# DDMAL/text_alignment

Hardware: AMD Instinct MI355X
Metric: nw_dp_cells_per_s (higher is better)
Workload: dtype int32; 1 GPU; affine-gap NW, 4096 problems of 4096x4096 per GPU per step, default scoring [8,-4,-7,-7,-3,0], two-phase (score fill + windowed traceback); parallelism=problems sharded x1, no data-path collective, distinct_problems=256

## Files before the change

### text_alignment_amd/csrc/nw_band.h

```cpp
#pragma once
#include <stdint.h>

#include "nw_cell.h"

namespace ta {

constexpr int kBandSentinel = -(1 << 24);
constexpr int kBandMaxLen = 32768;
static_assert(((int64_t)kBandSentinel - 2ll * kBandMaxLen * 128 - (1 << 21)) * 64 > INT32_MIN, "sentinel-derived values, encoded");
struct BandRange { int gl, gh; };
TA_HD BandRange band_groups(int n, int m, int w, int s) {
    const int ngroups = PtrLayout<4>::ngroups(m);
    const int lo = (m < n ? m - n : 0) - w, hi = (m > n ? m - n : 0) + w;
    const int i0 = s * 256 + 1;
    const int jmin = i0 + lo > 1 ? i0 + lo : 1;
    const int jmax = i0 + 255 + hi < m ? i0 + 255 + hi : m;
    const int kmin = jmin - 1, kmax = jmax - 1 + 63;
    int gl = kmin >= 2 ? ((kmin - 2) / 64) * 16 - 16 : 0;
    if (gl < 0) gl = 0;
    int gh = (kmax / 64) * 16 + 32;
    if (gh >= ngroups || gh <= gl) gh = ngroups;
    if (gl >= gh) gl = 0;
    return BandRange{gl, gh};
}
// ... 51 lines not shown
    const int off_lo = m < n ? m - n : 0, off_hi = m > n ? m - n : 0;
    const int lo = wl < w_outer ? off_lo - (int)wl : off_lo - w_outer;
    const int hi = wh < w_outer ? off_hi + (int)wh : off_hi + w_outer;
    const int i0 = s * 256 + 1;
    const int jmin = i0 + lo > 1 ? i0 + lo : 1;
    const int jmax = i0 + 255 + hi < m ? i0 + 255 + hi : m;
    const int kmin = jmin - 1, kmax = jmax - 1 + 63;
    int gl = kmin >= 2 ? ((kmin - 2) / 64) * 16 - 16 : 0;
    if (gl < 0) gl = 0;
    int gh = (kmax / 64) * 16 + 32;
    if (gh >= ngroups || gh <= gl) gh = ngroups;
    if (gl >= gh) gl = 0;
    return BandRange{gl, gh};
}
template <int PM = kFunnelFullPm>
TA_HD bool funnel_ok(int n, int m, const FunnelSys& f, int w_outer) {
    const int nstrips = PtrLayout<4>::nstrips(n), ngroups = PtrLayout<4>::ngroups(m);
    BandRange prev{0, 0};
    for (int s = 0; s < nstrips; ++s) {
        const BandRange r = funnel_raw<PM>(n, m, f, w_outer, s);
        if (r.gl < 0) return false;
        if (s > 0) {
            if (r.gl < prev.gl || r.gh < prev.gh) return false;
            if (r.gl > 0 && prev.gh < ngroups && 4 * r.gl + 2 > 4 * prev.gh - 63) return false;
        }
        prev = r;
    }
    return true;
}
TA_HD BandRange funnel_groups(int n, int m, const int32_t* prm, int w_outer, int s) {
    const FunnelSys f = funnel_sys(prm);
    return funnel_ok(n, m, f, w_outer) ? funnel_raw(n, m, f, w_outer, s) : band_groups(n, m, w_outer, s);
}
template <int PM = kFunnelFullPm>
inline bool funnel_ranges(int n, int m, const int32_t* prm, int w_outer, BandRange* rg) {
    const FunnelSys f = funnel_sys(prm);
    const bool own = funnel_ok<PM>(n, m, f, w_outer);
    const int nstrips = PtrLayout<4>::nstrips(n);
    for (int s = 0; s < nstrips; ++s) rg[s] = own ? funnel_raw<PM>(n, m, f, w_outer, s) : band_groups(n, m, w_outer, s);
    return own;
}

TA_HD int funnel_jlo(const BandRange& r, int i) { return r.gl == 0 ? 1 : 4 * r.gl - ((i - 1) % 256) / 4 + 3; }
TA_HD int funnel_jhi(const BandRange& r, int i, int m) {
    if (r.gh == PtrLayout<4>::ngroups(m)) return m;
    const int j = 4 * r.gh - ((i - 1) % 256) / 4;
    return j < m ? j : m;
}
inline int64_t funnel_exit0(int n, int m, const int32_t* prm, const BandRange* rg) {
    const FunnelSys f = funnel_sys(prm);
    int64_t best = -(1ll << 40);
    auto out = [&](int i, int j) {
        if (i < 1 || i > n || j < 1 || j > m) return false;
        const BandRange& r = rg[(i - 1) / 256];
        return j < funnel_jlo(r, i) || j > funnel_jhi(r, i, m);
    };
    auto take = [&](int64_t db, int i, int j) {
        if (out(i, j)) best = bmax(best, db + f.ap + funnel_suf<int64_t>(n - i, m - j, f));
    };
    for (int j = 0; j <= m; ++j) { take(-j, 1, j); take(-j, 1, j + 1); }
    for (int i = 1; i <= n; ++i) { take(-i, i, 1); take(-i, i + 1, 1); }
    return best;
}

struct FunnelLcs { int mat, mis; };
TA_HD FunnelLcs funnel_lcs_sys(const int32_t* prm) { return FunnelLcs{prm[0], prm[1]}; }
template <typename T>
TA_HD T funnel_suf_lcs(T rn, T rm, T l, const FunnelSys& f, const FunnelLcs& q) {
    const T stat = funnel_suf<T>(rn, rm, f);
    if (q.mis >= q.mat) return stat;
    const T d = rn < rm ? rn : rm;
    const T lp = l < d ? (l < 0 ? 0 : l) : d;
    const T none = rn * (T)f.cvi + rm * (T)f.chi;
    const T all_match = lp * (T)q.mat + (rn - lp) * (T)f.cvi + (rm - lp) * (T)f.chi;
    const T most = lp * (T)q.mat + (d - lp) * (T)q.mis + (rn - d) * (T)f.cvi + (rm - d) * (T)f.chi;
    T best = none > all_match ? none : all_match;
    if (most > best) best = most;
    return best < stat ? best : stat;
}

constexpr int kLcsMaxM = 4096;
constexpr int kLcsMaxAlphabet = 64;

TA_HD int lcs_row_off(int max_n) { return (max_n + 1 + 63) & ~63; }
TA_HD int64_t lcs_stride(int max_n) { return (int64_t)lcs_row_off(max_n) + 192ll * PtrLayout<4>::nstrips(max_n); }
TA_HD int lcs_row_at(const int32_t* row, int m, int j) {
    const int c = m - j;
    if (c <= 0) return 0;
    const int w = c >> 6, b = c & 63;
    if (w >= 64) return row[128 + 63] + __builtin_popcountll(((const uint64_t*)row)[63]);
    const uint64_t bits = ((const uint64_t*)row)[w];
    return row[128 + w] + (b ? __builtin_popcountll(bits & ((1ull << b) - 1)) : 0);
}

struct LcsRun { int t0, w, s, l, b, count; };
struct LcsRunCursor { int s, l; };
TA_HD LcsRunCursor lcs_run_begin(int n) { return LcsRunCursor{PtrLayout<4>::nstrips(n), -1}; }
template <typename GhOf>
TA_HD LcsRun lcs_next_run(int n, int m, int ngroups, LcsRunCursor& c, GhOf&& gh_of) {
    while (true) {
        if (c.l < 0) {
            if (--c.s < 0) return LcsRun{INT32_MAX, 0, 0, 0, 0, 0};
            const int top = (n - 256 * c.s - 1) >> 2;
            c.l = top < 63 ? top : 63;
        }
        const int gh = gh_of(c.s);
        const int lmin = 4 * gh > m ? 4 * gh - m : 0;
        if (gh >= ngroups || c.l < lmin) { c.l = -1; continue; }
        const int cnt = m - 4 * gh + c.l, b = cnt & 63, left = c.l - lmin + 1;
        const LcsRun r{n - 256 * c.s - 4 * c.l - 1 + (cnt >> 6), cnt >> 6, c.s, c.l, b, b + 1 < left ? b + 1 : left};
        c.l = r.count == left ? -1 : c.l - r.count;
        return r;
    }
}

}
```

### text_alignment_amd/csrc/ta_nw2.hip

```cpp
#include <hip/hip_runtime.h>
#include <stdint.h>
#include <array>
#include <atomic>
#include <map>
#include <type_traits>
#include <vector>

#include "nw_band.h"
#include "nw_cell.h"
#include "nw_hw.h"
#include "ta_common.h"

namespace ta {

#ifndef TA_CK_GROUPS
#define TA_CK_GROUPS 16
#endif
constexpr int kCkGroups = TA_CK_GROUPS;
static_assert(kCkGroups % 4 == 0 && kCkGroups >= 4, "whole blocks of four groups");
constexpr int kStateInts = 10;
constexpr int kWsRange = 0x7ffff000;

#ifndef TA_SUBROWS
#define TA_SUBROWS 2
// ... 483 lines not shown
                            rowp[col] = make_int2(kBandSentinel, kBandSentinel);
                    }
                }
                if (W > 1) {
                    asm volatile("s_waitcnt vmcnt(0)" ::: "memory");
                    if (lane == 63)
                        __hip_atomic_store(&prog[wave], pass * ngroups + ngroups, __ATOMIC_RELEASE,
                                           __HIP_MEMORY_SCOPE_WORKGROUP);
                }
            }
        }
        for (; g < g_fin; ++g) group_edge(g);
        patch(false);
    }
    if constexpr (FUNNEL) {
        if (lane == 0 && cnt_wave > 0) {
            atomicMax(&a.band_cert[kCertWords * p + 1], ex_wave);
            atomicAdd(&a.band_cert[kCertWords * p + 2], cnt_wave);
        }
    }
}

__global__ __launch_bounds__(256) void nw_band_cert_init_kernel(NwArgs a, const int32_t* x0) {
    const int p = blockIdx.x * 256 + threadIdx.x;
    if (p >= a.nprob) return;
    const int n = (int)(a.t_off[p + 1] - a.t_off[p]), m = (int)(a.o_off[p + 1] - a.o_off[p]);
    const bool own = n > 0 && m > 0 && n <= kBandMaxLen && m <= kBandMaxLen &&
                     funnel_ok(n, m, funnel_sys(a.params + (size_t)p * a.params_stride), a.band_w);
    a.band_cert[kCertWords * p] = INT32_MIN;
    a.band_cert[kCertWords * p + 1] = x0[p];
    a.band_cert[kCertWords * p + 2] = 0;
    a.band_cert[kCertWords * p + 3] = own ? 1 : 0;
    a.band_ok[p] = 0;
}
__global__ __launch_bounds__(256) void nw_band_certify_kernel(NwArgs a) {
    const int p = blockIdx.x * 256 + threadIdx.x;
    if (p >= a.nprob) return;
    const int n = (int)(a.t_off[p + 1] - a.t_off[p]);
    const int32_t* c = a.band_cert + kCertWords * (size_t)p;
    const bool ok = n > 0 && c[2] == PtrLayout<4>::nstrips(n) && c[0] > a.band_u[p] && c[0] > c[1];
    a.band_ok[p] = ok ? 1 : 0;
}

__global__ __launch_bounds__(256) void nw_band_cert_init_lcs_kernel(NwArgs a, const int32_t* x0, int alphabet) {
    const int p = blockIdx.x * 256 + threadIdx.x;
    if (p >= a.nprob) return;
    const int n = (int)(a.t_off[p + 1] - a.t_off[p]), m = (int)(a.o_off[p + 1] - a.o_off[p]);
    const int32_t* prm = a.params + (size_t)p * a.params_stride;
    const FunnelSys f = funnel_sys(prm);
    const bool sized = n > 0 && m > 0 && n <= kBandMaxLen && m <= kBandMaxLen;
    const bool lcs = sized && n >= 2 && m <= kLcsMaxM && n <= a.lcs_max_n && alphabet > 0 && alphabet <= kLcsMaxAlphabet &&
                     prm[0] > prm[1] && funnel_ok<kFunnelLcsScalePm>(n, m, f, a.band_w);
    const bool own = lcs || (sized && funnel_ok(n, m, f, a.band_w));
    a.band_cert[kCertWords * p] = INT32_MIN;
    a.band_cert[kCertWords * p + 1] = lcs ? -(1 << 30) : x0[p];
    a.band_cert[kCertWords * p + 2] = lcs ? -1 : 0;
    a.band_cert[kCertWords * p + 3] = lcs ? 2 : own ? 1 : 0;
    a.band_ok[p] = 0;
}

#ifndef TA_LCS_PROFILE
#define TA_LCS_PROFILE 0
#endif
#if TA_LCS_PROFILE
#define LCS_PROFILE_DECL long long pc_t = __builtin_readcyclecounter(), pc_setup = 0, pc_steps = 0, pc_events = 0, pc_tail = 0;
#define LCS_LAP(acc) { const long long now_ = __builtin_readcyclecounter(); acc += now_ - pc_t; pc_t = now_; }
#else
#define LCS_PROFILE_DECL
#define LCS_LAP(acc)
#endif
constexpr int kLcsUnroll = 3;
static_assert(63 % kLcsUnroll == 0, "nw_lcs_suffix_kernel: 63 steps in whole iterations, the 64th swaps the feed");
__global__ __launch_bounds__(64) void nw_lcs_suffix_kernel(NwArgs a, int alphabet) {
    extern __shared__ __attribute__((aligned(16))) unsigned char smem[];
    const int p = blockIdx.x;
    if (a.band_cert[kCertWords * p + 3] != 2) return;
    const int64_t t0 = a.t_off[p], o0 = a.o_off[p];
    const int n = (int)(a.t_off[p + 1] - t0), m = (int)(a.o_off[p + 1] - o0);
    const int32_t* prm = a.params + (size_t)p * a.params_stride;
    const FunnelSys fsys = funnel_sys(prm);
    const FunnelLcs lsys = funnel_lcs_sys(prm);
    const int lane = threadIdx.x;
    const int nstrips = PtrLayout<4>::nstrips(n), ngroups = PtrLayout<4>::ngroups(m);
    uint64_t* const mask = reinterpret_cast<uint64_t*>(smem);
    int* const rg = reinterpret_cast<int*>(smem + (size_t)(alphabet + 1) * 512);
    int32_t* const out = a.lcs + (size_t)p * lcs_stride(a.lcs_max_n);
    int32_t* const rows = out + lcs_row_off(a.lcs_max_n);
    LCS_PROFILE_DECL

    for (int k = 0; k <= alphabet; ++k) mask[k * 64 + lane] = 0;
    for (int b0 = 0; b0 < 64; b0 += 16) {
        int syms[16];
#pragma unroll
        for (int k = 0; k < 16; ++k) {
            const int c = 64 * lane + b0 + k;
            syms[k] = c < m ? a.o_codes[o0 + m - 1 - c] : -1;
        }
#pragma unroll
        for (int k = 0; k < 16; ++k)
            if ((unsigned)syms[k] < (unsigned)alphabet) mask[syms[k] * 64 + lane] |= 1ull << (b0 + k);
    }
    for (int s = lane; s < nstrips; s += 64) {
        const BandRange r = funnel_raw<kFunnelLcsScalePm>(n, m, fsys, a.band_w, s);
        rg[2 * s] = r.gl; rg[2 * s + 1] = r.gh;
    }
    for (int k = lane; k < 64 * nstrips; k += 64) out[k] = 0;
    __threadfence();
    __syncthreads();
    auto is_out = [&](int i, int j) {
        if (i < 1 || i > n || j < 1 || j > m) return false;
        const BandRange r{rg[2 * ((i - 1) / 256)], rg[2 * ((i - 1) / 256) + 1]};
        return j < funnel_jlo(r, i) || j > funnel_jhi(r, i, m);
    };
    auto exit0 = [&](int db, int i2, int j2, int l) {
        return db + fsys.ap + funnel_suf_lcs<int>(n - i2, m - j2, l, fsys, lsys);
    };

    LcsRunCursor ev_c = lcs_run_begin(n);
    int ev_t, ev_n, ev_w, ev_b, ev_k;
    auto next_run = [&]() __attribute__((always_inline)) {
        const LcsRun r = lcs_next_run(n, m, ngroups, ev_c, [&](int s) { return __builtin_amdgcn_readfirstlane(rg[2 * s + 1]); });
        ev_t = r.t0; ev_n = r.count; ev_w = r.w; ev_b = r.b; ev_k = 64 * r.s + r.l;
    };
    next_run();
    int row_t = n - 256 * (nstrips - 1) - 1, row_d = 0;
    int32_t* row_p = rows + 192 * (nstrips - 1);
    int nx_t = min(ev_t, row_t);

    const int pad = alphabet * 512;
    const unsigned char* const mask_lane = smem + lane * 8;
    auto load_feed = [&](int base) {
        const int tk = n - 1 - base - lane;
        int f = pad;
        if (tk >= 0) { const int c = a.t_codes[t0 + tk]; f = (unsigned)c < (unsigned)alphabet ? c * 512 : pad; }
        return f;
    };
    uint64_t V = ~0ull;
    int cy = 0, nc = 0, ex = -(1 << 30);
    int feed = load_feed(0);
    int symn = __builtin_amdgcn_update_dpp(feed, pad, 0x138, 0xf, 0xf, false);
    uint64_t Mn = *reinterpret_cast<const uint64_t*>(mask_lane + symn);
    const int nchunks = (n + 63 + 63) / 64;
    LCS_LAP(pc_setup)
    auto stores = [&](int t, int nin) __attribute__((always_inline)) {
        LCS_LAP(pc_steps)
        if (t == ev_t) {
            if (lane == ev_w) out[ev_k] = 64 * ev_w - nin + __builtin_popcountll(~V & ((1ull << ev_b) - 1));
            if (--ev_n > 0) { ev_t += 4; --ev_k; --ev_b; } else next_run();
        }
        if (t == row_t) {
            if (lane == row_d) {
                reinterpret_cast<uint64_t*>(row_p)[lane] = ~V;
                row_p[128 + lane] = 64 * lane - nin;
            }
            ++row_t;
            if (++row_d == 64) {
                row_d = 0; row_t += 192; row_p -= 192;
                if (row_p < rows) row_t = INT32_MAX;
            }
        }
        nx_t = min(ev_t, row_t);
        LCS_LAP(pc_events)
    };
    auto step = [&](int t) __attribute__((always_inline)) {
        const int sym = symn;
        const uint64_t M = Mn;
        symn = __builtin_amdgcn_update_dpp(feed, sym, 0x138, 0xf, 0xf, false);
        Mn = *reinterpret_cast<const uint64_t*>(mask_lane + symn);
        const int cin = __builtin_amdgcn_update_dpp(0, cy, 0x138, 0xf, 0xf, true);
        const int nin = __builtin_amdgcn_update_dpp(0, nc, 0x138, 0xf, 0xf, true);
        const uint64_t U = V & M;
        const uint64_t sum = V + U + (uint64_t)(unsigned)cin;
        const uint32_t sh = (uint32_t)(sum >> 32), uh = (uint32_t)(U >> 32), vh = (uint32_t)(V >> 32);
        cy = (int)(((sh & uh) | (~sh & vh)) >> 31);
        V = sum | (V & ~M);
        nc = nin + __builtin_popcountll(V);
        if (__builtin_expect(t == nx_t, 0)) stores(t, nin);
    };
    for (int ch = 0; ch < nchunks; ++ch) {
        const int base = ch * 64;
        const int feed_next = load_feed(base + 64);
        LCS_LAP(pc_tail)
#pragma unroll 1
        for (int q = 0; q < 63; q += kLcsUnroll) {
#pragma unroll
            for (int k = 0; k < kLcsUnroll; ++k) {
                feed = __builtin_amdgcn_update_dpp(feed, feed, 0x134, 0xf, 0xf, false);
                step(base + q + k);
            }
        }
        feed = feed_next;
        step(base + 63);
        LCS_LAP(pc_steps)
        const int ltot = 64 * 64 - __builtin_amdgcn_readlane(nc, 63);
        const int r = base + 1 - lane, i = n - r;
        if (r >= 0 && r <= n) {
            if (is_out(i, 1)) ex = max(ex, exit0(-i, i, 1, ltot));
            if (is_out(i + 1, 1)) ex = max(ex, exit0(-i, i + 1, 1, ltot));
        }
    }
    LCS_LAP(pc_tail)
    const int pc = 64 * (lane + 1) - nc;
    {
        const int before = pc - __builtin_popcountll(~V);
        for (int b = 0; b < 64; ++b) {
            const int cnt = 64 * lane + b, j = m - cnt;
            if (j < 0) break;
            const int l = before + (b ? __builtin_popcountll(~V & ((1ull << b) - 1)) : 0);
            if (is_out(1, j)) ex = max(ex, exit0(-j, 1, j, l));
            if (is_out(1, j + 1)) ex = max(ex, exit0(-j, 1, j + 1, l));
        }
    }
    ex = wave_max_i32(ex);
    if (lane == 0) {
        atomicMax(&a.band_cert[kCertWords * p + 1], ex);
        __threadfence();
        atomicAdd(&a.band_cert[kCertWords * p + 2], 1);
#if TA_LCS_PROFILE
        const int spare = 64 * PtrLayout<4>::nstrips(a.lcs_max_n);
        if (lcs_row_off(a.lcs_max_n) - spare >= 8) {
            long long* const pc = reinterpret_cast<long long*>(out + spare);
            pc[0] = pc_setup; pc[1] = pc_steps; pc[2] = pc_events; pc[3] = pc_tail;
        }
#endif
    }
}

constexpr int kChunk = kCkGroups;
constexpr int kChunkGroups = kChunk + 1;
constexpr int kChunkSteps = kChunkGroups * 4;
#ifndef TA_TB2_LANES
#define TA_TB2_LANES 32
#endif
constexpr int kWinLanes = TA_TB2_LANES;
static_assert(kWinLanes >= 8 && kWinLanes <= 64, "window lanes");
constexpr int kHalfLanes = 32;
static_assert(kSubRows == 2 && kSubLanes == kHalfLanes, "nw_trace2h_kernel restarts half-strips: phase 1 must keep lane 31's rows");

#ifndef TA_P2_PROFILE
#define TA_P2_PROFILE 0
#endif
#if TA_P2_PROFILE
#define PC_LAP(acc) { const long long now_ = __builtin_readcyclecounter(); acc += now_ - pc_t; pc_t = now_; }
#else
#define PC_LAP(acc)
#endif

__device__ __forceinline__ void wave_sync() {
    __builtin_amdgcn_fence(__ATOMIC_ACQ_REL, "wavefront");
    __builtin_amdgcn_wave_barrier();
}
// ... 663 lines not shown
        if (__all(T.done)) {
            if (lam == 0) tok_s[i % NWV][half][5] = 4;
            if (lane == 0) __hip_atomic_store(&seq_s, i + 1, __ATOMIC_RELEASE, __HIP_MEMORY_SCOPE_WORKGROUP);
            break;
        }
        const bool live = !T.done;
        const TbJob J = T.job;
        if (live && !tb_serves(spec, J)) refill_job<UL>(P, lds, J, lam);
        TbTok N = T;
        TbWalk& w = N.w;
        if (live) {
            const int lb = (J.u * UL) & 63, i_h = J.u * (R * UL);
            const int g0 = J.ck * kChunk;
            const int kvalid = J.ck > 0 ? g0 * SPG + 2 : 0;
            const int l = ((w.x - 1) % L::SR) / R, r = (w.x - 1) % R, k = (w.y - 1) + l;
            if (enter_chunk<UL>(P, lds, w, g0, kvalid, k, l - lb, r)) {
                w.len += walk_half(lds.win, g0, kvalid, i_h, lb, w.x, w.y, w.st, P.ops + (P.cap - 1 - w.len),
                                   P.cap - w.len, lam, half);
                if (w.st >= 3) { w.pend = w.st; w.st = 0; }
            }
        }
        N.job = live ? tb_job_at<UL>(w.x, w.y) : TbJob{-1, 0, 0, 0};
        N.done = !live || N.job.u < 0 || i >= max_iter_w;
        if (live && N.done) tb_finish(a, P, w.x, w.y, w.len, lam == 0);
        if (lam == 0) tok_store(tok_s[i % NWV][half], N);
        if (lane == 0) __hip_atomic_store(&seq_s, i + 1, __ATOMIC_RELEASE, __HIP_MEMORY_SCOPE_WORKGROUP);
        if (__all(N.done)) break;
        T = N;
        kt = i;
    }
}

}

using namespace ta;

extern "C" int32_t ta_nw2_max_m(void) { return 65000; }

extern "C" int64_t ta_nw2_workspace_bytes(int32_t n, int32_t m) {
    if (n <= 0 || m <= 0) return 16;
    return (Ws2(n, m).total + 15) & ~(int64_t)15;
}

template <int W, int MODE, bool SAMEGO, typename OC, int BAND = 0>
static hipError_t launch_score_k(const NwArgs& a, size_t lds, hipStream_t st) {
    hipError_t e = allow_full_lds(&nw_score_kernel<W, MODE, SAMEGO, OC, BAND>);
    if (e != hipSuccess) return e;
    hipLaunchKernelGGL((nw_score_kernel<W, MODE, SAMEGO, OC, BAND>), dim3(a.nprob), dim3(W * 64), lds, st, a);
    return hipGetLastError();
}

template <int W>
static hipError_t launch_score_band(const NwArgs& a, size_t lds, bool samego, hipStream_t st) {
    hipError_t e = hipMemsetAsync(a.band_ok, 0, sizeof(int32_t) * (size_t)a.nprob, st);
    if (e != hipSuccess) return e;
    e = samego ? launch_score_k<W, 2, true, uint16_t, 1>(a, lds, st) : launch_score_k<W, 2, false, uint16_t, 1>(a, lds, st);
    if (e != hipSuccess) return e;
    return samego ? launch_score_k<W, 2, true, uint16_t, 2>(a, lds, st) : launch_score_k<W, 2, false, uint16_t, 2>(a, lds, st);
}

template <int W>
static hipError_t launch_score_funnel(const NwArgs& a, const int32_t* x0, size_t lds, bool samego, hipStream_t st) {
    const dim3 grid((a.nprob + 255) / 256);
    hipLaunchKernelGGL(nw_band_cert_init_kernel, grid, dim3(256), 0, st, a, x0);
    hipError_t e = hipGetLastError();
    if (e != hipSuccess) return e;
    e = samego ? launch_score_k<W, 2, true, uint16_t, 3>(a, lds, st) : launch_score_k<W, 2, false, uint16_t, 3>(a, lds, st);
    if (e != hipSuccess) return e;
    hipLaunchKernelGGL(nw_band_certify_kernel, grid, dim3(256), 0, st, a);
    e = hipGetLastError();
    if (e != hipSuccess) return e;
    return samego ? launch_score_k<W, 2, true, uint16_t, 2>(a, lds, st) : launch_score_k<W, 2, false, uint16_t, 2>(a, lds, st);
}

template <int W>
static hipError_t launch_score_funnel_lcs(const NwArgs& a, const int32_t* x0, size_t lds, bool samego, int alphabet,
                                          hipStream_t st) {
    const dim3 grid((a.nprob + 255) / 256);
    const bool covers = alphabet > 0 && alphabet <= kLcsMaxAlphabet;
    hipLaunchKernelGGL(nw_band_cert_init_lcs_kernel, grid, dim3(256), 0, st, a, x0, covers ? alphabet : 0);
    hipError_t e = hipGetLastError();
    if (e != hipSuccess) return e;
    if (covers) {
        const size_t lcs_lds = (size_t)(alphabet + 1) * 512 + 8 * (size_t)PtrLayout<4>::nstrips(a.lcs_max_n);
        hipLaunchKernelGGL(nw_lcs_suffix_kernel, dim3(a.nprob), dim3(64), lcs_lds, st, a, alphabet);
        e = hipGetLastError();
        if (e != hipSuccess) return e;
    }
    e = samego ? launch_score_k<W, 2, true, uint16_t, 4>(a, lds, st) : launch_score_k<W, 2, false, uint16_t, 4>(a, lds, st);
    if (e != hipSuccess) return e;
    hipLaunchKernelGGL(nw_band_certify_kernel, grid, dim3(256), 0, st, a);
    e = hipGetLastError();
    if (e != hipSuccess) return e;
    return samego ? launch_score_k<W, 2, true, uint16_t, 2>(a, lds, st) : launch_score_k<W, 2, false, uint16_t, 2>(a, lds, st);
}

template <int W>
static hipError_t launch_score_w(const NwArgs& a, size_t lds, bool profile, bool samego, bool codes8, hipStream_t st) {
    if (profile) return samego ? launch_score_k<W, 2, true, uint16_t>(a, lds, st)
                               : launch_score_k<W, 2, false, uint16_t>(a, lds, st);
    return codes8 ? launch_score_k<W, 1, false, uint8_t>(a, lds, st)
                  : launch_score_k<W, 1, false, uint16_t>(a, lds, st);
}

constexpr size_t kLdsShared = 124 * 1024;
struct P1Plan { int mode, w, apad; size_t lds; bool samego, codes8; };

static P1Plan plan_phase1(int max_n, int max_m, uint32_t flags, int nprob = 1 << 20) {
    P1Plan pl{};
    const int nstrips = PtrLayout<4>::nstrips(max_n);
    const int wmax = nstrips >= 8 ? 8 : nstrips >= 4 ? 4 : nstrips >= 2 ? 2 : 1;
    pl.codes8 = (flags & TA_NW_CODES8) != 0;
    pl.samego = (flags & TA_NW_OPENS_SAME) != 0;
    const int alphabet = (int)((flags >> TA_NW_ALPHABET_SHIFT) & 0xFFu);
    bool profile = alphabet > 0 && alphabet < 255 && !(flags & TA_NW_NO_PROFILE);
    pl.w = wmax;
    const int ngroups = PtrLayout<4>::ngroups(max_m);
    auto choose = [&](auto lds_of, int w_least, int& w_out) -> int {
        int best_w = 0, best_res = 0;
        double best_score = 0.0;
        for (int cand : {4, 8, 2, 1}) {
            if (cand > wmax || cand < w_least) continue;
            const size_t need = lds_of(cand);
            if (need > 160 * 1024) continue;
            const int res = (int)std::min<size_t>(kLdsShared / need, 20 / cand) * cand;
            const int passes = (nstrips + cand - 1) / cand;
            const double busy = (double)passes * ngroups / ((double)passes * ngroups + 25.0 * (cand - 1));
            const double fill = std::min(1.0, (double)nprob * cand / (256.0 * 12.0));
            const double score = std::min(res, 12) * busy * fill;
            if (score > best_score + 1e-9) { best_score = score; best_res = res; best_w = cand; }
        }
        w_out = best_w;
        return best_res;
    };
    if (profile) {
        pl.apad = alphabet + 1;
        int w = 0;
        const int res = choose([&](int cand) { return P1Lds(max_m, 2, cand * pl.apad * 256).total; }, 1, w);
        if (w == 0 || res < 8) profile = false;
        else pl.w = w;
    }
    if (!profile) {
        int w = 0;
        choose([&](int) { return P1Lds(max_m, pl.codes8 ? 1 : 2).total; }, std::min(4, wmax), w);
        if (w > 0) pl.w = w;
    }
    if (const int v = (int)((flags >> TA_NW_WAVES_SHIFT) & 0xFu)) {
        if ((v == 1 || v == 2 || v == 4 || v == 8) && v <= wmax &&
            (!profile || P1Lds(max_m, 2, v * pl.apad * 256).total <= 160 * 1024))
            pl.w = v;
    }
    pl.mode = profile ? 2 : 1;
    if (!profile) pl.apad = 0;
    pl.lds = profile ? P1Lds(max_m, 2, pl.w * pl.apad * 256).total : P1Lds(max_m, pl.codes8 ? 1 : 2).total;
    return pl;
}

extern "C" int ta_nw2_phase1_plan_batch(int32_t max_n, int32_t max_m, int32_t nprob, uint32_t flags, int32_t* out) {
    if (!out || max_n < 0 || max_m < 0 || nprob < 0) return ta_fail(TA_EINVAL, "bad argument");
    const P1Plan pl = plan_phase1(max_n, max_m, flags, nprob);
    out[0] = pl.mode; out[1] = pl.w; out[2] = (int32_t)pl.lds; out[3] = pl.samego ? 1 : 0;
    return TA_OK;
}

extern "C" int ta_nw2_phase1_plan(int32_t max_n, int32_t max_m, uint32_t flags, int32_t* out) {
    return ta_nw2_phase1_plan_batch(max_n, max_m, 1 << 20, flags, out);
}

static int32_t clamp_i32(int64_t v) { return (int32_t)std::max<int64_t>(-(1ll << 30), std::min<int64_t>(v, 1ll << 30)); }

extern "C" int32_t ta_nw2_band_bound(int32_t n, int32_t m, const int32_t* params, int32_t w) {
    if (!params || n < 0 || m < 0 || w < 0) return INT32_MAX;
    return clamp_i32(band_bound(n, m, params, w));
}

constexpr int kBandThetaNum = 1, kBandThetaDen = 2;
static int band_rule_w(int n, int m, const int32_t* prm) {
    const int64_t a = std::max(prm[0], prm[1]);
    const int64_t cv = std::max<int64_t>((int64_t)prm[4] + std::max(prm[2], 0), -1);
    const int64_t ch = std::max<int64_t>((int64_t)prm[5] + std::max(prm[3], 0), -1);
    if (a <= 0 || a - cv - ch <= 0) return -1;
    const int64_t target = a * std::min(n, m) * kBandThetaNum;
    int lo = 0, hi = std::max(n, m);
    if (band_bound(n, m, prm, hi) * kBandThetaDen >= target) return -1;
    while (lo < hi) {
        const int mid = lo + (hi - lo) / 2;
        if (band_bound(n, m, prm, mid) * kBandThetaDen < target) hi = mid; else lo = mid + 1;
    }
    return lo;
}
static void band_share(int n, int m, int w, int64_t& run, int64_t& all) {
    const int nstrips = PtrLayout<4>::nstrips(n), ngroups = PtrLayout<4>::ngroups(m);
    run = 0; all = (int64_t)nstrips * ngroups;
    for (int s = 0; s < nstrips; ++s) { const BandRange r = band_groups(n, m, w, s); run += r.gh - r.gl; }
}
constexpr int kBandMinN = 1024;
constexpr int kBandMaxSharePermille = 800;

extern "C" int ta_nw2_band_plan(const int32_t* n_arr, const int32_t* m_arr, int32_t nprob, const int32_t* params,
                                int32_t params_stride, uint32_t flags, int32_t band, int32_t* out, int32_t* u_out,
                                int32_t* ranges_out, int32_t ranges_cap) {
    if (!n_arr || !m_arr || !params || !out || nprob < 0 || band < 0 || (params_stride != 0 && params_stride != 6))
        return ta_fail(TA_EINVAL, "bad argument");
    for (int k = 0; k < 6; ++k) out[k] = 0;
    out[1] = -1;
    if (nprob == 0) return TA_OK;
    int big = 0, max_n = 0, max_m = 0;
    for (int p = 0; p < nprob; ++p) {
        if (n_arr[p] < 0 || m_arr[p] < 0) return ta_fail(TA_EINVAL, "negative size");
        if ((int64_t)n_arr[p] * m_arr[p] > (int64_t)n_arr[big] * m_arr[big]) big = p;
        max_n = std::max(max_n, n_arr[p]); max_m = std::max(max_m, m_arr[p]);
    }
    out[4] = big;
    out[3] = PtrLayout<4>::nstrips(n_arr[big]);
    int w_rule = 0;
    for (int p = 0; p < nprob && w_rule >= 0; ++p) {
        if (n_arr[p] <= 0 || m_arr[p] <= 0) continue;
        if (params_stride == 0 && p > 0 && n_arr[p] == n_arr[p - 1] && m_arr[p] == m_arr[p - 1]) continue;
        const int wp = band_rule_w(n_arr[p], m_arr[p], params + (size_t)p * params_stride);
        w_rule = wp < 0 ? -1 : std::max(w_rule, wp);
    }
    out[1] = w_rule;
    const P1Plan pl = plan_phase1(max_n, max_m, flags, nprob);
    const bool can = pl.mode == 2 && (pl.w == 4 || pl.w == 8) && max_n <= kBandMaxLen && max_m <= kBandMaxLen &&
                     n_arr[big] > 0 && m_arr[big] > 0;
    int w_use = 0;
    int64_t run = 0, all = 1;
    if (w_rule >= 0) band_share(n_arr[big], m_arr[big], std::max(w_rule, 2), run, all);
    if (band >= 2) w_use = can ? band : 0;
    else if (band == 0 && can && w_rule >= 0 && max_n >= kBandMinN && run * 1000 < all * kBandMaxSharePermille)
        w_use = std::max(w_rule, 2);
    if (w_use > 0) band_share(n_arr[big], m_arr[big], w_use, run, all);
    out[0] = w_use;
    const bool funnel = w_use > 0 && band == 0;
    const int32_t* prm_big = params + (size_t)big * params_stride;
    std::vector<BandRange> rg_big((size_t)out[3]);
    if (funnel) {
        funnel_ranges(n_arr[big], m_arr[big], prm_big, w_use, rg_big.data());
        run = 0;
        for (const BandRange& r : rg_big) run += r.gh - r.gl;
        out[5] = 1;
    }
    out[2] = (int32_t)(run * 1000 / all);
    const int w_show = w_use > 0 ? w_use : std::max(w_rule, 0);
    if (ranges_out)
        for (int s = 0; s < out[3] && 2 * s + 1 < ranges_cap; ++s) {
            const BandRange r = funnel ? rg_big[s] : band_groups(n_arr[big], m_arr[big], w_show, s);
            ranges_out[2 * s] = r.gl; ranges_out[2 * s + 1] = r.gh;
        }
    if (u_out && w_use > 0)
        for (int p = 0; p < nprob; ++p)
            u_out[p] = (params_stride == 0 && p > 0 && n_arr[p] == n_arr[p - 1] && m_arr[p] == m_arr[p - 1])
                           ? u_out[p - 1]
                           : clamp_i32(band_bound(n_arr[p], m_arr[p], params + (size_t)p * params_stride, w_use));
    return TA_OK;
}

extern "C" int32_t ta_nw2_funnel_suf(int32_t rn, int32_t rm, const int32_t* params, int32_t* ap_out) {
    if (!params || rn < 0 || rm < 0) return INT32_MAX;
    const FunnelSys f = funnel_sys(params);
    if (ap_out) *ap_out = f.ap;
    return clamp_i32(funnel_suf<int64_t>(rn, rm, f));
}

extern "C" int ta_nw2_funnel_plan(const int32_t* n_arr, const int32_t* m_arr, int32_t nprob, const int32_t* params,
                                  int32_t params_stride, int32_t w, int32_t big, int32_t* x0_out, int32_t* ranges_out,
                                  int32_t ranges_cap, int32_t* out) {
    if (!n_arr || !m_arr || !params || nprob < 0 || w < 2 || (params_stride != 0 && params_stride != 6) ||
        (nprob > 0 && (big < 0 || big >= nprob)))
        return ta_fail(TA_EINVAL, "bad argument");
    std::vector<BandRange> rg;
    std::map<std::array<int32_t, 8>, int32_t> x0_of;
    for (int p = 0; p < nprob; ++p) {
        const int n = n_arr[p], m = m_arr[p];
        if (n < 0 || m < 0 || n > kBandMaxLen || m > kBandMaxLen) return ta_fail(TA_EINVAL, "size outside the band's range");
        if (n == 0 || m == 0) { if (x0_out) x0_out[p] = 0; continue; }
        const int32_t* prm = params + (size_t)p * params_stride;
        const std::array<int32_t, 8> key{n, m, prm[0], prm[1], prm[2], prm[3], prm[4], prm[5]};
        const auto hit = x0_of.find(key);
        if (hit != x0_of.end() && p != big) { if (x0_out) x0_out[p] = hit->second; continue; }
        rg.resize(PtrLayout<4>::nstrips(n));
        const bool own = funnel_ranges(n, m, prm, w, rg.data());
        const int32_t x0 = hit != x0_of.end() ? hit->second : clamp_i32(funnel_exit0(n, m, prm, rg.data()));
        x0_of[key] = x0;
        if (x0_out) x0_out[p] = x0;
        if (p == big) {
            int64_t run = 0;
            for (size_t s = 0; s < rg.size(); ++s) {
                run += rg[s].gh - rg[s].gl;
                if (ranges_out && 2 * (int)s + 1 < ranges_cap) { ranges_out[2 * s] = rg[s].gl; ranges_out[2 * s + 1] = rg[s].gh; }
            }
            if (out) {
                out[0] = own ? 1 : 0;
                out[1] = (int32_t)(run * 1000 / ((int64_t)rg.size() * PtrLayout<4>::ngroups(m)));
            }
        }
    }
    return TA_OK;
}

static hipError_t launch_score(NwArgs a, int max_n, int max_m, uint32_t flags, hipStream_t st, const int32_t* band_x0 = nullptr) {
    const P1Plan pl = plan_phase1(max_n, max_m, flags, a.nprob);
    if (pl.lds > 160 * 1024) return hipErrorInvalidValue;
    a.apad = pl.apad;
    if (a.band_w > 0) {
        if (pl.mode != 2 || !a.band_u || !a.band_ok) return hipErrorInvalidValue;
        if (a.band_cert) {
            if (!band_x0) return hipErrorInvalidValue;
            if (a.lcs) {
                const int alphabet = (int)((flags >> TA_NW_ALPHABET_SHIFT) & 0xFFu);
                if (pl.w == 8) return launch_score_funnel_lcs<8>(a, band_x0, pl.lds, pl.samego, alphabet, st);
                if (pl.w == 4) return launch_score_funnel_lcs<4>(a, band_x0, pl.lds, pl.samego, alphabet, st);
                return hipErrorInvalidValue;
            }
            if (pl.w == 8) return launch_score_funnel<8>(a, band_x0, pl.lds, pl.samego, st);
            if (pl.w == 4) return launch_score_funnel<4>(a, band_x0, pl.lds, pl.samego, st);
            return hipErrorInvalidValue;
        }
        if (pl.w == 8) return launch_score_band<8>(a, pl.lds, pl.samego, st);
        if (pl.w == 4) return launch_score_band<4>(a, pl.lds, pl.samego, st);
        return hipErrorInvalidValue;
    }
    switch (pl.w) {
    case 8: return launch_score_w<8>(a, pl.lds, pl.mode == 2, pl.samego, pl.codes8, st);
    case 4: return launch_score_w<4>(a, pl.lds, pl.mode == 2, pl.samego, pl.codes8, st);
    case 2: return launch_score_w<2>(a, pl.lds, pl.mode == 2, pl.samego, pl.codes8, st);
    default: return launch_score_w<1>(a, pl.lds, pl.mode == 2, pl.samego, pl.codes8, st);
    }
}

extern "C" int32_t ta_nw2_traceback_plan(int32_t nprob, int32_t params_stride, uint32_t flags) {
    const int tbw = (int)((flags >> TA_NW_TBWAVES_SHIFT) & 0x7u);
    if (tbw >= 1 && tbw <= 6) return tbw;
    if (nprob <= 832) return 4;
    if (params_stride != 0) return nprob <= 1088 ? 2 : nprob <= 1600 ? 4 : 1;
    if (nprob <= 1088) return 6;
    if (nprob <= 2560) return 5;
    return 3;
}

__global__ __launch_bounds__(256) void nw_check_ids_kernel(NwArgs a, int bound, int* bad) {
    const int p = blockIdx.x;
    int mine = 0;
    for (int64_t i = a.t_off[p] + threadIdx.x; i < a.t_off[p + 1]; i += 256) mine |= (unsigned)a.t_codes[i] >= (unsigned)bound;
    for (int64_t i = a.o_off[p] + threadIdx.x; i < a.o_off[p + 1]; i += 256) mine |= (unsigned)a.o_codes[i] >= (unsigned)bound;
    if (__ballot(mine) != 0 && (threadIdx.x & 63) == 0) atomicOr(bad, 1);
}

static int check_ids(const NwArgs& a, uint32_t flags, hipStream_t st) {
    int bound = 65535;
    if (flags & TA_NW_CODES8) bound = 255;
    const int alpha = (int)((flags >> TA_NW_ALPHABET_SHIFT) & 0xFFu);
    if (alpha > 0 && !(flags & TA_NW_NO_PROFILE)) bound = alpha < bound ? alpha : bound;
    int* bad = nullptr;
    hipError_t e = hipMallocAsync(reinterpret_cast<void**>(&bad), sizeof(int), st);
    if (e != hipSuccess) return ta_fail_hip(e, "TA_NW_CHECK_IDS: hipMallocAsync");
    int host_bad = 0;
    e = hipMemsetAsync(bad, 0, sizeof(int), st);
    if (e == hipSuccess) {
        hipLaunchKernelGGL(nw_check_ids_kernel, dim3(a.nprob), dim3(256), 0, st, a, bound, bad);
        e = hipGetLastError();
    }
    if (e == hipSuccess) e = hipMemcpyAsync(&host_bad, bad, sizeof(int), hipMemcpyDeviceToHost, st);
    (void)hipFreeAsync(bad, st);
    if (e == hipSuccess) e = hipStreamSynchronize(st);
    if (e != hipSuccess) return ta_fail_hip(e, "TA_NW_CHECK_IDS");
    if (host_bad) return ta_fail(TA_EINVAL, "a token id is outside the range the flags assert (TA_NW_CODES8 / TA_NW_ALPHABET)");
    return TA_OK;
}

extern "C" int ta_nw2_batch(const int32_t* t_codes, const int64_t* t_off,
                            const int32_t* o_codes, const int64_t* o_off, int32_t nprob,
                            const int32_t* params, int32_t params_stride,
                            uint8_t* ws, const int64_t* ws_off,
                            uint8_t* ops_out, const int64_t* ops_off, int32_t* ops_len,
                            int32_t max_n, int32_t max_m, int64_t score_bound,
                            uint32_t flags, void* stream) {
    return ta_nw2_batch_band(t_codes, t_off, o_codes, o_off, nprob, params, params_stride, ws, ws_off, ops_out, ops_off,
                             ops_len, max_n, max_m, score_bound, flags, 0, nullptr, nullptr, stream);
}

extern "C" int ta_nw2_batch_band(const int32_t* t_codes, const int64_t* t_off,
                                 const int32_t* o_codes, const int64_t* o_off, int32_t nprob,
                                 const int32_t* params, int32_t params_stride,
                                 uint8_t* ws, const int64_t* ws_off,
// ... 104 lines not shown
```

Baseline: 8579 billion cells/s.

## Split LCS suffix mask into two-level hi/lo rows and relax planner for forced band

The LCS suffix kernel's per-symbol bitmask table, one LDS row per alphabet symbol, is replaced by a factored table of (alphabet/8)+1 high rows and 8 low rows. Each symbol's mask becomes the AND of one high row and one low row, and the table is built with LDS atomic ORs. This caps LDS per one-wave workgroup so more workgroups fit per CU at any alphabet size. The cost is two LDS loads plus an AND per step instead of one load, and atomics during setup. Separately, the phase-1 planner can fall back to a smaller group width when a band is forced, so a banded kernel path is kept instead of disabling the profile.

```diff
diff --git a/text_alignment_amd/csrc/nw_band.h b/text_alignment_amd/csrc/nw_band.h
--- a/text_alignment_amd/csrc/nw_band.h
+++ b/text_alignment_amd/csrc/nw_band.h
@@ -157,6 +157,22 @@
 constexpr int kLcsMaxM = 4096;
 constexpr int kLcsMaxAlphabet = 64;
 
+constexpr int kLcsMaskRowBytes = 512;
+TA_HD int lcs_mask_hi_rows(int alphabet) { return (alphabet + 7) >> 3; }
+TA_HD int lcs_mask_rows(int alphabet) { return lcs_mask_hi_rows(alphabet) + 1 + 8; }
+TA_HD uint32_t lcs_mask_offsets(int code, int alphabet) {
+    const int nhi = lcs_mask_hi_rows(alphabet);
+    const bool in = (unsigned)code < (unsigned)alphabet;
+    const uint32_t hi = in ? (uint32_t)code >> 3 : (uint32_t)nhi, lo = (uint32_t)nhi + 1 + (in ? (uint32_t)code & 7 : 0);
+    return (hi * kLcsMaskRowBytes) << 16 | lo * kLcsMaskRowBytes;
+}
+TA_HD uint32_t lcs_mask_pad(int alphabet) { return lcs_mask_offsets(-1, alphabet); }
+TA_HD size_t lcs_mask_lds_bytes(int alphabet, int max_n) {
+    return (size_t)lcs_mask_rows(alphabet) * kLcsMaskRowBytes + 8 * (size_t)PtrLayout<4>::nstrips(max_n);
+}
+static_assert((kLcsMaxAlphabet + 7) / 8 + 1 + 8 == 17 && 17 * kLcsMaskRowBytes + 8 * ((kBandMaxLen + 255) / 256) <= 10240,
+              "nw_lcs_suffix_kernel: 16 one-wave workgroups per CU at every alphabet and height it takes");
+
 TA_HD int lcs_row_off(int max_n) { return (max_n + 1 + 63) & ~63; }
 TA_HD int64_t lcs_stride(int max_n) { return (int64_t)lcs_row_off(max_n) + 192ll * PtrLayout<4>::nstrips(max_n); }
 TA_HD int lcs_row_at(const int32_t* row, int m, int j) {
diff --git a/text_alignment_amd/csrc/ta_nw2.hip b/text_alignment_amd/csrc/ta_nw2.hip
--- a/text_alignment_amd/csrc/ta_nw2.hip
+++ b/text_alignment_amd/csrc/ta_nw2.hip
@@ -589,13 +589,15 @@
     const FunnelLcs lsys = funnel_lcs_sys(prm);
     const int lane = threadIdx.x;
     const int nstrips = PtrLayout<4>::nstrips(n), ngroups = PtrLayout<4>::ngroups(m);
+    const int mask_rows = lcs_mask_rows(alphabet);
     uint64_t* const mask = reinterpret_cast<uint64_t*>(smem);
-    int* const rg = reinterpret_cast<int*>(smem + (size_t)(alphabet + 1) * 512);
+    int* const rg = reinterpret_cast<int*>(smem + (size_t)mask_rows * kLcsMaskRowBytes);
+    unsigned char* const mask_lane = smem + lane * 8;
     int32_t* const out = a.lcs + (size_t)p * lcs_stride(a.lcs_max_n);
     int32_t* const rows = out + lcs_row_off(a.lcs_max_n);
     LCS_PROFILE_DECL
 
-    for (int k = 0; k <= alphabet; ++k) mask[k * 64 + lane] = 0;
+    for (int k = 0; k < mask_rows; ++k) mask[k * 64 + lane] = 0;
     for (int b0 = 0; b0 < 64; b0 += 16) {
         int syms[16];
 #pragma unroll
@@ -604,8 +606,14 @@
             syms[k] = c < m ? a.o_codes[o0 + m - 1 - c] : -1;
         }
 #pragma unroll
-        for (int k = 0; k < 16; ++k)
-            if ((unsigned)syms[k] < (unsigned)alphabet) mask[syms[k] * 64 + lane] |= 1ull << (b0 + k);
+        for (int k = 0; k < 16; ++k) {
+            const uint32_t off = lcs_mask_offsets(syms[k], alphabet);
+            const uint64_t bit = (unsigned)syms[k] < (unsigned)alphabet ? 1ull << (b0 + k) : 0;
+            __hip_atomic_fetch_or(reinterpret_cast<uint64_t*>(mask_lane + (off >> 16)), bit, __ATOMIC_RELAXED,
+                                  __HIP_MEMORY_SCOPE_WORKGROUP);
+            __hip_atomic_fetch_or(reinterpret_cast<uint64_t*>(mask_lane + (off & 0xffffu)), bit, __ATOMIC_RELAXED,
+                                  __HIP_MEMORY_SCOPE_WORKGROUP);
+        }
     }
     for (int s = lane; s < nstrips; s += 64) {
         const BandRange r = funnel_raw<kFunnelLcsScalePm>(n, m, fsys, a.band_w, s);
@@ -634,19 +642,21 @@
     int32_t* row_p = rows + 192 * (nstrips - 1);
     int nx_t = min(ev_t, row_t);
 
-    const int pad = alphabet * 512;
-    const unsigned char* const mask_lane = smem + lane * 8;
+    const int pad = (int)lcs_mask_pad(alphabet);
+    typedef __attribute__((address_space(3))) unsigned char lds_byte;
+    typedef __attribute__((address_space(3))) const uint64_t lds_word;
+    const uint32_t lane8 = (uint32_t)(uintptr_t)(lds_byte*)smem + lane * 8;
+    auto row_a = [&](int pk) { return *(lds_word*)(uintptr_t)(((uint32_t)pk >> 16) + lane8); };
+    auto row_b = [&](int pk) { return *(lds_word*)(uintptr_t)(((uint32_t)pk & 0xffffu) + lane8); };
     auto load_feed = [&](int base) {
         const int tk = n - 1 - base - lane;
-        int f = pad;
-        if (tk >= 0) { const int c = a.t_codes[t0 + tk]; f = (unsigned)c < (unsigned)alphabet ? c * 512 : pad; }
-        return f;
+        return tk >= 0 ? (int)lcs_mask_offsets(a.t_codes[t0 + tk], alphabet) : pad;
     };
     uint64_t V = ~0ull;
     int cy = 0, nc = 0, ex = -(1 << 30);
     int feed = load_feed(0);
     int symn = __builtin_amdgcn_update_dpp(feed, pad, 0x138, 0xf, 0xf, false);
-    uint64_t Mn = *reinterpret_cast<const uint64_t*>(mask_lane + symn);
+    uint64_t An = row_a(symn), Bn = row_b(symn);
     const int nchunks = (n + 63 + 63) / 64;
     LCS_LAP(pc_setup)
     auto stores = [&](int t, int nin) __attribute__((always_inline)) {
@@ -671,9 +681,9 @@
     };
     auto step = [&](int t) __attribute__((always_inline)) {
         const int sym = symn;
-        const uint64_t M = Mn;
+        const uint64_t M = An & Bn;
         symn = __builtin_amdgcn_update_dpp(feed, sym, 0x138, 0xf, 0xf, false);
-        Mn = *reinterpret_cast<const uint64_t*>(mask_lane + symn);
+        An = row_a(symn); Bn = row_b(symn);
         const int cin = __builtin_amdgcn_update_dpp(0, cy, 0x138, 0xf, 0xf, true);
         const int nin = __builtin_amdgcn_update_dpp(0, nc, 0x138, 0xf, 0xf, true);
         const uint64_t U = V & M;
@@ -1503,7 +1513,7 @@
     hipError_t e = hipGetLastError();
     if (e != hipSuccess) return e;
     if (covers) {
-        const size_t lcs_lds = (size_t)(alphabet + 1) * 512 + 8 * (size_t)PtrLayout<4>::nstrips(a.lcs_max_n);
+        const size_t lcs_lds = lcs_mask_lds_bytes(alphabet, a.lcs_max_n);
         hipLaunchKernelGGL(nw_lcs_suffix_kernel, dim3(a.nprob), dim3(64), lcs_lds, st, a, alphabet);
         e = hipGetLastError();
         if (e != hipSuccess) return e;
@@ -1527,7 +1537,7 @@
 constexpr size_t kLdsShared = 124 * 1024;
 struct P1Plan { int mode, w, apad; size_t lds; bool samego, codes8; };
 
-static P1Plan plan_phase1(int max_n, int max_m, uint32_t flags, int nprob = 1 << 20) {
+static P1Plan plan_phase1(int max_n, int max_m, uint32_t flags, int nprob = 1 << 20, bool band_forced = false) {
     P1Plan pl{};
     const int nstrips = PtrLayout<4>::nstrips(max_n);
     const int wmax = nstrips >= 8 ? 8 : nstrips >= 4 ? 4 : nstrips >= 2 ? 2 : 1;
@@ -1558,7 +1568,12 @@
         pl.apad = alphabet + 1;
         int w = 0;
         const int res = choose([&](int cand) { return P1Lds(max_m, 2, cand * pl.apad * 256).total; }, 1, w);
-        if (w == 0 || res < 8) profile = false;
+        if (w != 0 && res < 8 && band_forced) {
+            w = 0;
+            choose([&](int cand) { return P1Lds(max_m, 2, cand * pl.apad * 256).total; }, 4, w);
+            if (w != 0) pl.w = w;
+            else profile = false;
+        } else if (w == 0 || res < 8) profile = false;
         else pl.w = w;
     }
     if (!profile) {
@@ -1642,7 +1657,7 @@
         w_rule = wp < 0 ? -1 : std::max(w_rule, wp);
     }
     out[1] = w_rule;
-    const P1Plan pl = plan_phase1(max_n, max_m, flags, nprob);
+    const P1Plan pl = plan_phase1(max_n, max_m, flags, nprob, band >= 2);
     const bool can = pl.mode == 2 && (pl.w == 4 || pl.w == 8) && max_n <= kBandMaxLen && max_m <= kBandMaxLen &&
                      n_arr[big] > 0 && m_arr[big] > 0;
     int w_use = 0;
@@ -1721,7 +1736,7 @@
 }
 
 static hipError_t launch_score(NwArgs a, int max_n, int max_m, uint32_t flags, hipStream_t st, const int32_t* band_x0 = nullptr) {
-    const P1Plan pl = plan_phase1(max_n, max_m, flags, a.nprob);
+    const P1Plan pl = plan_phase1(max_n, max_m, flags, a.nprob, a.band_w > 0);
     if (pl.lds > 160 * 1024) return hipErrorInvalidValue;
     a.apad = pl.apad;
     if (a.band_w > 0) {
```

Result: faster. 9023 billion cells/s (median of 6 runs) (+5.2%).
